# E-J408/admm-net

Measured on AMD Instinct MI355X. Metric: signals/sec (K-layer ADMM-Net forward), higher is better.
Workload: dtype f32; 1 GPU; cfg3: ADMMNet K=16 grid 16x16 (D=256, n=257) batch 65536/GPU + spectrum on 1024 atoms; batch_per_gpu=65536, global_batch=65536, K=16, D=256, n=257, natoms=1024, batch_mean_scope=global, chunk=8192, weights=torch.manual_seed(0) default init, glayer=matrix function, checked per matrix; eigensolver on the rejected matrices

## Files before the change

### admm_net_amd/csrc/spectral_fused.hip

```cpp
#include <stdio.h>
#include <stdlib.h>

#include <type_traits>

#include "common.h"
#include "rebuild_core.h"
#include "lane_reduce.h"

namespace admmnet {

constexpr int SF_THREADS = 768, SF_WAVES = 12;
constexpr int SF_PITCH = 40;
constexpr int SF_MAXM = 4;

typedef __bf16 bf16x8 __attribute__((ext_vector_type(8)));
typedef __bf16 bf16x2 __attribute__((ext_vector_type(2)));
typedef float f32x2v __attribute__((ext_vector_type(2)));
using f32x16 = __attribute__((ext_vector_type(16))) float;

__device__ __forceinline__ unsigned sf_pack_bf16(float a, float b) {
    const f32x2v p = {a, b};
    return __builtin_bit_cast(unsigned, __builtin_convertvector(p, bf16x2));
}
__device__ __forceinline__ float sf_bf16_lo(unsigned u) { return __uint_as_float(u << 16); }
__device__ __forceinline__ float sf_bf16_hi(unsigned u) { return __uint_as_float(u & 0xffff0000u); }

__device__ __forceinline__ float sf_reduce4(float a, float b, float c, float d) {
    float a2 = a, c2 = c, b2 = b, d2 = d;
    asm volatile("s_nop 1\n\tv_permlane32_swap_b32 %0, %1\n\tv_permlane32_swap_b32 %2, %3\n\ts_nop 1"
                 : "+v"(a2), "+v"(c2), "+v"(b2), "+v"(d2));
    float x = a2 + c2, y = b2 + d2;
    asm volatile("s_nop 1\n\tv_permlane16_swap_b32 %0, %1\n\ts_nop 1" : "+v"(x), "+v"(y));
    return pn_row16_sum(x + y);
}

template <int W>
__device__ __forceinline__ void sf_block_sum4(float &a, float &b, float &c, float &d, float *red ) {
    const float t = sf_reduce4(a, b, c, d);
    const int lane = threadIdx.x & 63, wave = threadIdx.x >> 6;
    __syncthreads();
    if ((lane & 15) == 0) red[(lane >> 4) * W + wave] = t;
    __syncthreads();
    float s[4];
#pragma unroll
    for (int q = 0; q < 4; ++q) {
        float v = 0.f;
#pragma unroll
        for (int w = 0; w < W; ++w) v += red[q * W + w];
        s[q] = v;
    }
    a = s[0]; b = s[1]; c = s[2]; d = s[3];
}

template <int W>
__device__ __forceinline__ void sf_block_sum8(float &a, float &b, float &c, float &d, float &e, float &f, float *red ) {
    const float t = sf_reduce4(a, b, c, d), u = sf_reduce4(e, f, 0.f, 0.f);
    const int lane = threadIdx.x & 63, wave = threadIdx.x >> 6;
    __syncthreads();
    if ((lane & 15) == 0) {
        red[(lane >> 4) * W + wave] = t;
        red[(4 + (lane >> 4)) * W + wave] = u;
    }
    __syncthreads();
    float s[6];
#pragma unroll
    for (int q = 0; q < 6; ++q) {
        float v = 0.f;
#pragma unroll
        for (int w = 0; w < W; ++w) v += red[q * W + w];
        s[q] = v;
    }
    a = s[0]; b = s[1]; c = s[2]; d = s[3]; e = s[4]; f = s[5];
}

struct SfCarve {
    int NP, NJ;
    float2 *X0, *X1, *Y0, *Y1, *ph, *Ob;
    float *hh, *hp, *red, *coef;
    double *sc;
    int *flags;
    float2 *part;
    unsigned short *ETre;
    unsigned short *ETim;
    __host__ __device__ static int np_of(int n) { return (n + 7) & ~7; }
    __host__ __device__ static int nj_of(int n) {
        const int D = n - 1, nt = (D + 31) >> 5;
        const int a = 32 * nt, b = (n + 7) & ~7;
        return a > b ? a : b;
    }
    __host__ __device__ static size_t bytes(int n, int W) {
        const size_t NP = np_of(n), NJ = nj_of(n);
        const size_t fixed = sizeof(float2) * 6 * NP + sizeof(float) * 2 * NP + sizeof(float) * 96 + sizeof(float) * 16 +
                             sizeof(double) * 16 + sizeof(int) * 4;
        const size_t part = sizeof(float2) * W * 2 * NP;
        const size_t slab = sizeof(unsigned short) * 2 * NJ * SF_PITCH;
        return fixed + (part > slab ? part : slab) + 64;
    }
    __device__ SfCarve(char *smem, int n) {
        NP = np_of(n);
        NJ = nj_of(n);
        sc = reinterpret_cast<double *>(smem);
        X0 = reinterpret_cast<float2 *>(sc + 16);
        X1 = X0 + NP; Y0 = X1 + NP; Y1 = Y0 + NP; ph = Y1 + NP; Ob = ph + NP;
        hh = reinterpret_cast<float *>(Ob + NP);
        hp = hh + NP;
        red = hp + NP;
        coef = red + 96;
        flags = reinterpret_cast<int *>(coef + 16);
        const int fixed = (int)(sizeof(double) * 16 + sizeof(float2) * 6 * NP + sizeof(float) * 2 * NP + sizeof(float) * 112 +
                                sizeof(int) * 4);
        char *u = smem + ((fixed + 15) & ~15);
        part = reinterpret_cast<float2 *>(u);
        ETre = reinterpret_cast<unsigned short *>(u);
        ETim = ETre + NJ * SF_PITCH;
    }
};

struct SfUpdate {
    const float *alpha;
    const float2 *phi_prev;
    const float *h_prev;
    const float *lw_prev;
    int mode;
};

__device__ __forceinline__ float2 sf_a_elem(int i, int j, int D, float2 z, float ir, float corner, float hi, float2 phj) {
    float2 a = make_float2(-ir * z.x, -ir * z.y);
    if (i < D) {
        if (i == j) a = make_float2(hi - ir * z.x, 0.f);
    } else {
        a = (j == D) ? make_float2(corner - ir * z.x, 0.f) : make_float2(phj.x - ir * z.x, -phj.y - ir * z.y);
    }
    return a;
}

template <int TPW, int W>
__global__ __launch_bounds__(64 * W, W == 12 ? 1 : 3) void sp_fused_kernel(int D, const float *__restrict__ lw, const float2 *__restrict__ phi,
                                                                 const float *__restrict__ h, float2 *Zg,
                                                                 float2 *G, float *__restrict__ rn,
                                                                 int *__restrict__ flag, int32_t *__restrict__ status, float tol,
                                                                 int iters, unsigned long long *__restrict__ ptime, SfUpdate up) {
    extern __shared__ __attribute__((aligned(16))) char smem[];
    long long t_prev = ptime ? clock64() : 0;
    auto mark = [&](int id) {
        if (ptime && threadIdx.x == 0) {
            const long long t_now = clock64();
            atomicAdd(&ptime[id], (unsigned long long)(t_now - t_prev));
            t_prev = t_now;
        }
    };
    const int n = D + 1;
    const SfCarve cv(smem, n);
    const int NP = cv.NP;
    const int64_t b = blockIdx.x;
    float2 *Z = Zg + b * (int64_t)n * n;
    const float2 *Gold = G + b * (int64_t)n * n;
    const int tid = threadIdx.x, lane = tid & 63;
    const int wave = __builtin_amdgcn_readfirstlane(tid >> 6);
    const float ir = lw[S_INV_RHO_G], corner = lw[S_CORNER_G];
    const int NT = (D + 31) >> 5, ntri = NT * (NT + 1) / 2;
    const int MM = (n + 63) >> 6;

    float pn = 0.f;
    if (tid < NP) {
        const float2 p = tid < D ? phi[b * D + tid] : make_float2(0.f, 0.f);
        cv.ph[tid] = p;
        cv.hh[tid] = tid < D ? h[b * D + tid] : 0.f;
        pn = p.x * p.x + p.y * p.y;
        if (up.mode) {
            cv.Ob[tid] = tid < D ? up.phi_prev[b * D + tid] : make_float2(0.f, 0.f);
            cv.hp[tid] = tid < D ? up.h_prev[b * D + tid] : 0.f;
        }
    }
    const float al = up.mode ? up.alpha[b] : 0.f;
    const float corner_zp = up.mode ? up.lw_prev[S_CORNER_Z] : 0.f;
    {
        float z1 = 0.f, z2 = 0.f, z3 = 0.f;
        sf_block_sum4<W>(pn, z1, z2, z3, cv.red);
    }
    const float ipn = pn > 0.f ? rsqrtf(pn) : 0.f;
    if (tid < NP) {
        const float2 p = cv.ph[tid];
        cv.X0[tid] = make_float2(tid == D ? 1.f : 0.f, 0.f);
        cv.X1[tid] = pn > 0.f ? make_float2(p.x * ipn, p.y * ipn) : make_float2(tid == 0 ? 1.f : 0.f, 0.f);
    }
    __syncthreads();

    mark(0);
    double trace = 0.0;
    float l0 = 0.f, l1 = 0.f, cf = 0.f, res0 = 0.f, res1 = 0.f;
    bool last = false;
    for (int it = 0; it < iters; ++it) {
        v2f x0[SF_MAXM], x1[SF_MAXM], c0[SF_MAXM], c1[SF_MAXM];
#pragma unroll
        for (int m = 0; m < SF_MAXM; ++m) {
            const int j = lane + 64 * m;
            const bool v = m < MM && j < n;
            x0[m] = v ? pk2(cv.X0[j]) : v2f{0.f, 0.f};
            x1[m] = v ? pk2(cv.X1[j]) : v2f{0.f, 0.f};
            c0[m] = v2f{0.f, 0.f};
            c1[m] = v2f{0.f, 0.f};
        }
        float trl = 0.f;
        auto run_pass = [&](auto updc) {
        constexpr bool UPD = decltype(updc)::value;
        float2 za[SF_MAXM], zb[SF_MAXM], zc[SF_MAXM], zd[SF_MAXM];
        float2 ga[SF_MAXM], gb[SF_MAXM], gc[SF_MAXM], gd[SF_MAXM];
        auto load_row = [&](int i, float2(&z)[SF_MAXM], float2(&g)[SF_MAXM]) {
#pragma unroll
            for (int m = 0; m < SF_MAXM; ++m) {
                const int j = lane + 64 * m;
                const bool v = i < n && j <= i;
                z[m] = (v && !(UPD && up.mode == 2)) ? Z[(int64_t)i * n + j] : make_float2(0.f, 0.f);
                if (UPD) g[m] = v ? Gold[(int64_t)i * n + j] : make_float2(0.f, 0.f);
            }
        };
        auto proc_row = [&](int i, float2(&zc)[SF_MAXM], const float2(&gq)[SF_MAXM]) {
            if (UPD) {
                const float hpi = cv.hp[i];
#pragma unroll
                for (int m = 0; m < SF_MAXM; ++m) {
                    if (64 * m <= i) {
                        const int j = lane + 64 * m;
                        if (j <= i) {
                            float2 c;
                            if (i < D) c = make_float2(i == j ? hpi : 0.f, 0.f);
                            else if (j == D) c = make_float2(corner_zp, 0.f);
                            else {
                                const float2 pp = cv.Ob[j];
                                c = make_float2(pp.x, -pp.y);
                            }
                            const float2 zn = make_float2(zc[m].x + al * (gq[m].x - c.x), zc[m].y + al * (gq[m].y - c.y));
                            zc[m] = zn;
                            Z[(int64_t)i * n + j] = zn;
                        }
                    }
                }
            }
            const v2f xi0 = pk2(cv.X0[i]), xi1 = pk2(cv.X1[i]);
            const float hi = cv.hh[i];
            v2f r0 = {0.f, 0.f}, r1 = {0.f, 0.f};
#pragma unroll
            for (int m = 0; m < SF_MAXM; ++m) {
                if (64 * m <= i) {
                    const int j = lane + 64 * m;
                    float2 a = sf_a_elem(i, j, D, zc[m], ir, corner, hi, (i == D && j < D) ? cv.ph[j] : make_float2(0.f, 0.f));
                    if (j > i) a = make_float2(0.f, 0.f);
                    if (j == i) trl += a.x;
                    const v2f av = pk2(a);
                    r0 = pk_cfma(r0, av, x0[m]);
                    r1 = pk_cfma(r1, av, x1[m]);
                    const v2f ac = (j < i) ? av : v2f{0.f, 0.f};
                    c0[m] = pk_cfma_conj(c0[m], ac, xi0);
                    c1[m] = pk_cfma_conj(c1[m], ac, xi1);
                }
            }
            if (i == 64 * SF_MAXM && lane == 0) {
                const int64_t idx = (int64_t)i * n + i;
                float2 z = (UPD && up.mode == 2) ? make_float2(0.f, 0.f) : Z[idx];
                if (UPD) {
                    const float2 g = Gold[idx];
                    z = make_float2(z.x + al * (g.x - corner_zp), z.y + al * g.y);
                    Z[idx] = z;
                }
                const float a = corner - ir * z.x;
                trl += a;
                const float2 xa = cv.X0[i], xb = cv.X1[i];
                r0.x += a * xa.x; r0.y += a * xa.y;
                r1.x += a * xb.x; r1.y += a * xb.y;
            }
            const float t = sf_reduce4(r0.x, r0.y, r1.x, r1.y);
            if ((lane & 15) == 0) {
                float *dst = reinterpret_cast<float *>((lane & 32) ? cv.Y1 : cv.Y0);
                dst[2 * i + ((lane >> 4) & 1)] = t;
            }
        };
        load_row(wave, za, ga);
        load_row(wave + W, zb, gb);
        for (int i = wave; i < n; i += 2 * W) {
            load_row(i + 2 * W, zc, gc);
            load_row(i + 3 * W, zd, gd);
            proc_row(i, za, ga);
            if (i + W < n) proc_row(i + W, zb, gb);
#pragma unroll
            for (int m = 0; m < SF_MAXM; ++m) {
                za[m] = zc[m];
                zb[m] = zd[m];
                ga[m] = gc[m];
                gb[m] = gd[m];
            }
        }
        };
        if (up.mode != 0 && it == 0) run_pass(std::true_type{});
        else run_pass(std::false_type{});
#pragma unroll
        for (int m = 0; m < SF_MAXM; ++m) {
            const int j = lane + 64 * m;
            if (m < MM && j < NP) {
                cv.part[(wave * 2 + 0) * NP + j] = make_float2(c0[m].x, c0[m].y);
                cv.part[(wave * 2 + 1) * NP + j] = make_float2(c1[m].x, c1[m].y);
            }
        }
        if (it == 0) {
            float z1 = 0.f, z2 = 0.f, z3 = 0.f;
            sf_block_sum4<W>(trl, z1, z2, z3, cv.red);
            trace = (double)trl;
        }
        __syncthreads();
        mark(1);
        float2 x0e = make_float2(0.f, 0.f), x1e = x0e, y0e = x0e, y1e = x0e;
        if (tid < n) {
            y0e = cv.Y0[tid];
            y1e = cv.Y1[tid];
#pragma unroll
            for (int w = 0; w < W; ++w) {
                if (tid >= 64 * SF_MAXM) break;
                const float2 p0 = cv.part[(w * 2 + 0) * NP + tid], p1 = cv.part[(w * 2 + 1) * NP + tid];
                y0e.x += p0.x; y0e.y += p0.y;
                y1e.x += p1.x; y1e.y += p1.y;
            }
            x0e = cv.X0[tid];
            x1e = cv.X1[tid];
        }
        float h00 = x0e.x * y0e.x + x0e.y * y0e.y, h11 = x1e.x * y1e.x + x1e.y * y1e.y;
        float h01r = x0e.x * y1e.x + x0e.y * y1e.y, h01i = x0e.x * y1e.y - x0e.y * y1e.x;
        sf_block_sum4<W>(h00, h11, h01r, h01i, cv.red);
        float ct = 1.f, st = 0.f, er = 1.f, ei = 0.f;
        {
            const float ab = sqrtf(h01r * h01r + h01i * h01i);
            const float dif = 0.5f * (h00 - h11), rad = sqrtf(dif * dif + ab * ab);
            l0 = 0.5f * (h00 + h11) - rad;
            l1 = 0.5f * (h00 + h11) + rad;
            const float vx = dif >= 0.f ? dif + rad : ab, vy = dif >= 0.f ? ab : rad - dif;
            const float nrm = sqrtf(vx * vx + vy * vy);
            if (nrm > 0.f) {
                ct = vx / nrm;
                st = vy / nrm;
            }
            if (ab > 0.f) {
                er = h01r / ab;
                ei = -h01i / ab;
            }
            cf = (float)((trace - (double)l0 - (double)l1) / (double)(n - 2));
            if (tid == 0) {
                cv.sc[0] = l0; cv.sc[1] = l1; cv.sc[2] = cf;
            }
        }
        const float2 ex1 = make_float2(er * x1e.x - ei * x1e.y, er * x1e.y + ei * x1e.x);
        const float2 ey1 = make_float2(er * y1e.x - ei * y1e.y, er * y1e.y + ei * y1e.x);
        const float2 nx0 = make_float2(-st * x0e.x + ct * ex1.x, -st * x0e.y + ct * ex1.y);
        const float2 nx1 = make_float2(ct * x0e.x + st * ex1.x, ct * x0e.y + st * ex1.y);
        const float2 ny0 = make_float2(-st * y0e.x + ct * ey1.x, -st * y0e.y + ct * ey1.y);
        const float2 ny1 = make_float2(ct * y0e.x + st * ey1.x, ct * y0e.y + st * ey1.y);
        const float2 d0 = make_float2(ny0.x - l0 * nx0.x, ny0.y - l0 * nx0.y);
        const float2 d1 = make_float2(ny1.x - l1 * nx1.x, ny1.y - l1 * nx1.y);
        float r0s = d0.x * d0.x + d0.y * d0.y, r1s = d1.x * d1.x + d1.y * d1.y;
        const float2 p0 = make_float2(ny0.x - cf * nx0.x, ny0.y - cf * nx0.y);
        const float2 p1 = make_float2(ny1.x - cf * nx1.x, ny1.y - cf * nx1.y);
        float n0 = p0.x * p0.x + p0.y * p0.y, n1 = p1.x * p1.x + p1.y * p1.y;
        float pr = p0.x * p1.x + p0.y * p1.y, pi = p0.x * p1.y - p0.y * p1.x;
        sf_block_sum8<W>(r0s, r1s, n0, n1, pr, pi, cv.red);
        res0 = sqrtf(r0s);
        res1 = sqrtf(r1s);
        last = it + 1 >= iters ||
               (it >= 1 && res0 <= 2e-6f * fabsf(l0 - cf) && res1 <= 2e-6f * fabsf(l1 - cf));
        if (!last) {
            const float in0 = n0 > 0.f ? rsqrtf(n0) : 0.f;
            const float2 q0 = make_float2(p0.x * in0, p0.y * in0);
            const float gr = pr * in0, gi = pi * in0;
            float2 q1 = make_float2(p1.x - (gr * q0.x - gi * q0.y), p1.y - (gr * q0.y + gi * q0.x));
            const float n1o = n1 - (gr * gr + gi * gi);
            const float in1 = n1o > 0.f ? rsqrtf(n1o) : 0.f;
            q1.x *= in1;
            q1.y *= in1;
            if (tid < NP) {
                cv.X0[tid] = tid < n ? q0 : make_float2(0.f, 0.f);
                cv.X1[tid] = tid < n ? q1 : make_float2(0.f, 0.f);
            }
        } else if (tid < NP) {
            cv.X0[tid] = tid < n ? nx0 : make_float2(0.f, 0.f);
            cv.X1[tid] = tid < n ? nx1 : make_float2(0.f, 0.f);
        }
        __syncthreads();
        mark(2);
        if (last) break;
    }
    const float mu0 = l0 - cf, mu1 = l1 - cf;

    int tI[TPW], tJ[TPW];
#pragma unroll
    for (int s = 0; s < TPW; ++s) tri_tile(wave * TPW + s, tI[s], tJ[s]);
    f32x16 accRe[TPW], accIm[TPW];
#pragma unroll
    for (int s = 0; s < TPW; ++s) {
#pragma unroll
        for (int q = 0; q < 16; ++q) {
            accRe[s][q] = 0.f;
            accIm[s][q] = 0.f;
        }
    }
    float2 ob = make_float2(0.f, 0.f);
    unsigned *ETre32 = reinterpret_cast<unsigned *>(cv.ETre), *ETim32 = reinterpret_cast<unsigned *>(cv.ETim);
    constexpr int P32 = SF_PITCH / 2;
    for (int idx = tid; idx < (cv.NJ - n) * P32; idx += (64 * W)) {
        ETre32[n * P32 + idx] = 0u;
        ETim32[n * P32 + idx] = 0u;
    }
    const int nslab = (n + 31) >> 5;
    for (int K = 0; K < nslab; ++K) {
        const int k0 = 32 * K;
        __syncthreads();
        int tl = tid;
        asm volatile("" : "+v"(tl));
        auto deflate = [&](float2 a, float2 vr0, float2 vc0, float2 vr1, float2 vc1, bool diag) {
            const float2 q0 = cmulc(vr0, vc0), q1 = cmulc(vr1, vc1);
            a.x -= mu0 * q0.x + mu1 * q1.x;
            a.y -= mu0 * q0.y + mu1 * q1.y;
            if (diag) {
                a.x -= cf;
                a.y = 0.f;
            }
            return a;
        };
        auto pair_of = [&](const float2 *v, int k, float2 &lo, float2 &hi) {
            const float4 t = *reinterpret_cast<const float4 *>(v + k);
            lo = make_float2(t.x, t.y);
            hi = make_float2(t.z, t.w);
        };
        {
            constexpr int RP = (64 * W) / 256, LQ = (16 + RP - 1) / RP;
            const int j = tl & 255;
            const float2 vj0 = cv.X0[j], vj1 = cv.X1[j], phj = cv.ph[j];
            constexpr int LB = 3;
#pragma unroll
            for (int qb = 0; qb < LQ; qb += LB) {
            float2 zl0[LB], zl1[LB];
#pragma unroll
            for (int uu = 0; uu < LB; ++uu) {
                const int kp = RP * (qb + uu) + (tl >> 8);
                const int k = k0 + 2 * kp;
                const bool v = kp < 16 && j <= k && j < n;
                zl0[uu] = (v && k < n) ? Z[(int64_t)k * n + j] : make_float2(0.f, 0.f);
                zl1[uu] = (v && k + 1 < n) ? Z[(int64_t)(k + 1) * n + j] : make_float2(0.f, 0.f);
            }
#pragma unroll
            for (int u = 0; u < LB; ++u) {
                const int kp = RP * (qb + u) + (tl >> 8);
                const int k = k0 + 2 * kp;
                if (kp < 16 && j <= k && j < n) {
                    float2 vk0, vk0b, vk1, vk1b;
                    pair_of(cv.X0, k, vk0, vk0b);
                    pair_of(cv.X1, k, vk1, vk1b);
                    const float2 hk = *reinterpret_cast<const float2 *>(cv.hh + k);
                    float2 e0 = make_float2(0.f, 0.f), e1 = e0;
                    if (k < n) e0 = deflate(sf_a_elem(k, j, D, zl0[u], ir, corner, hk.x, phj), vk0, vj0, vk1, vj1, k == j);
                    if (k + 1 < n) e1 = deflate(sf_a_elem(k + 1, j, D, zl1[u], ir, corner, hk.y, phj), vk0b, vj0, vk1b, vj1, k + 1 == j);
                    ETre32[j * P32 + kp] = sf_pack_bf16(e0.x, e1.x);
                    ETim32[j * P32 + kp] = sf_pack_bf16(e0.y, e1.y);
                }
            }
            }
        }
        if (tl < 16 && D >= 256) {
            const int kp = tl, k = k0 + 2 * kp, j = 256;
            if (j <= k && j < n) {
                float2 e0 = make_float2(0.f, 0.f);
                if (k < n)
                    e0 = deflate(sf_a_elem(k, j, D, Z[(int64_t)k * n + j], ir, corner, cv.hh[k], cv.ph[j]), cv.X0[k], cv.X0[j], cv.X1[k],
                                 cv.X1[j], k == j);
                ETre32[j * P32 + kp] = sf_pack_bf16(e0.x, 0.f);
                ETim32[j * P32 + kp] = sf_pack_bf16(e0.y, 0.f);
            }
        }
        {
            constexpr int RPS = (64 * W) / 16, UB = 2;
            const int kp = tl & 15, k = k0 + 2 * kp;
            const int kc = k < NP - 1 ? k : 0;
            float2 vk0, vk0b, vk1, vk1b, phk, phkb;
            pair_of(cv.X0, kc, vk0, vk0b);
            pair_of(cv.X1, kc, vk1, vk1b);
            pair_of(cv.ph, kc, phk, phkb);
            for (int jb = k0 + 1; jb < n; jb += UB * RPS) {
                float2 zu0[UB], zu1[UB];
#pragma unroll
                for (int u = 0; u < UB; ++u) {
                    const int j = jb + RPS * u + (tl >> 4);
                    const bool v = j < n && j >= k + 1;
                    zu0[u] = v ? Z[(int64_t)j * n + k] : make_float2(0.f, 0.f);
                    zu1[u] = (v && k + 1 < n) ? Z[(int64_t)j * n + k + 1] : make_float2(0.f, 0.f);
                }
#pragma unroll
                for (int u = 0; u < UB; ++u) {
                    const int j = jb + RPS * u + (tl >> 4);
                    if (j < n && j >= k + 1) {
                        const float hj = cv.hh[j];
                        const float2 vj0 = cv.X0[j], vj1 = cv.X1[j];
                        float2 e0 = deflate(sf_a_elem(j, k, D, zu0[u], ir, corner, hj, phk), vj0, vk0, vj1, vk1, false);
                        float2 e1 = make_float2(0.f, 0.f);
                        if (k + 1 < n)
                            e1 = deflate(sf_a_elem(j, k + 1, D, zu1[u], ir, corner, hj, phkb), vj0, vk0b, vj1, vk1b, j == k + 1);
                        ETre32[j * P32 + kp] = sf_pack_bf16(e0.x, e1.x);
                        ETim32[j * P32 + kp] = sf_pack_bf16(-e0.y, -e1.y);
                    }
                }
            }
        }
        __syncthreads();
        mark(3);
        {
            int r32 = lane & 31, kh = lane >> 5;
            asm volatile("" : "+v"(r32), "+v"(kh));
#pragma unroll
            for (int ks = 0; ks < 2; ++ks) {
                const int off = 8 * ks + 4 * kh;
                uint4 are = make_uint4(0, 0, 0, 0), aim = are;
#pragma unroll
                for (int s = 0; s < TPW; ++s) {
                    if (wave * TPW + s < ntri) {
                        const int ia = 32 * tI[s] + r32, jb_ = 32 * tJ[s] + r32;
                        if (s == 0 || tI[s] != tI[s - 1]) {
                            are = *reinterpret_cast<const uint4 *>(ETre32 + ia * P32 + off);
                            aim = *reinterpret_cast<const uint4 *>(ETim32 + ia * P32 + off);
                        }
                        const uint4 bre = *reinterpret_cast<const uint4 *>(ETre32 + jb_ * P32 + off);
                        const uint4 bim = *reinterpret_cast<const uint4 *>(ETim32 + jb_ * P32 + off);
                        const uint4 nbre = make_uint4(bre.x ^ 0x80008000u, bre.y ^ 0x80008000u, bre.z ^ 0x80008000u,
                                                      bre.w ^ 0x80008000u);
                        const bf16x8 Are = __builtin_bit_cast(bf16x8, are), Aim = __builtin_bit_cast(bf16x8, aim);
                        const bf16x8 Bre = __builtin_bit_cast(bf16x8, bre), Bim = __builtin_bit_cast(bf16x8, bim);
                        const bf16x8 nBre = __builtin_bit_cast(bf16x8, nbre);
                        accRe[s] = __builtin_amdgcn_mfma_f32_32x32x16_bf16(Are, Bre, accRe[s], 0, 0, 0);
                        accIm[s] = __builtin_amdgcn_mfma_f32_32x32x16_bf16(Are, Bim, accIm[s], 0, 0, 0);
                        accRe[s] = __builtin_amdgcn_mfma_f32_32x32x16_bf16(Aim, Bim, accRe[s], 0, 0, 0);
                        accIm[s] = __builtin_amdgcn_mfma_f32_32x32x16_bf16(Aim, nBre, accIm[s], 0, 0, 0);
                    }
                }
            }
        }
        mark(4);
        __syncthreads();
        if (tid < n) {
            const unsigned *dre = ETre32 + D * P32, *dim = ETim32 + D * P32;
            const unsigned *jre = ETre32 + tid * P32, *jim = ETim32 + tid * P32;
#pragma unroll 2
            for (int kp = 0; kp < 16; ++kp) {
                const unsigned ur = dre[kp], ui = dim[kp], vr = jre[kp], vi = jim[kp];
                const float ar0 = sf_bf16_lo(ur), ai0 = sf_bf16_lo(ui), br0 = sf_bf16_lo(vr), bi0 = sf_bf16_lo(vi);
                const float ar1 = sf_bf16_hi(ur), ai1 = sf_bf16_hi(ui), br1 = sf_bf16_hi(vr), bi1 = sf_bf16_hi(vi);
                {
                    asm volatile("v_fma_f32 %0, %1, %2, %0" : "+v"(ob.x) : "v"(ar0), "v"(br0));
                    asm volatile("v_fma_f32 %0, %1, %2, %0" : "+v"(ob.x) : "v"(ai0), "v"(bi0));
                    asm volatile("v_fma_f32 %0, %1, %2, %0" : "+v"(ob.x) : "v"(ar1), "v"(br1));
                    asm volatile("v_fma_f32 %0, %1, %2, %0" : "+v"(ob.x) : "v"(ai1), "v"(bi1));
                    asm volatile("v_fma_f32 %0, %1, %2, %0" : "+v"(ob.y) : "v"(ar0), "v"(bi0));
                    asm volatile("v_fma_f32 %0, -%1, %2, %0" : "+v"(ob.y) : "v"(ai0), "v"(br0));
                    asm volatile("v_fma_f32 %0, %1, %2, %0" : "+v"(ob.y) : "v"(ar1), "v"(bi1));
                    asm volatile("v_fma_f32 %0, -%1, %2, %0" : "+v"(ob.y) : "v"(ai1), "v"(br1));
                }
            }
        }
        mark(5);
    }
    __syncthreads();
    if (tid < NP) cv.Ob[tid] = tid < n ? ob : make_float2(0.f, 0.f);

    float fro = 0.f;
    {
        const int r32 = lane & 31, kh = lane >> 5;
#pragma unroll
        for (int s = 0; s < TPW; ++s) {
            if (wave * TPW + s < ntri) {
                const float wgt = tI[s] == tJ[s] ? 1.f : 2.f;
                const int gj = 32 * tJ[s] + r32;
#pragma unroll
                for (int q = 0; q < 16; ++q) {
                    const int gi = 32 * tI[s] + (q & 3) + 8 * (q >> 2) + 4 * kh;
                    if (gi < D && gj < D) fro += wgt * (accRe[s][q] * accRe[s][q] + accIm[s][q] * accIm[s][q]);
                }
            }
        }
        if (tid < n) fro += (tid < D ? 2.f : 1.f) * (ob.x * ob.x + ob.y * ob.y);
        float z1 = 0.f, z2 = 0.f, z3 = 0.f;
        sf_block_sum4<W>(fro, z1, z2, z3, cv.red);
    }
    const LayerLayout L{D};
    const float *vn = lw + L.off_vn();
    if (wave == 0) {
        const double thr = lw[S_THR];
        const double dl0 = cv.sc[0], dl1 = cv.sc[1], c = cv.sc[2];
        const double delta = sqrt(sqrt((double)fro)) * (1.0 + 0x1p-8);
        const double ts[9] = {-1.0, 0.0, 1.0, -0.75, -0.5, -0.25, 0.25, 0.5, 0.75};
        double arg = c;
        if (lane < 9) arg = c + ts[lane] * delta;
        else if (lane == 9) arg = dl0;
        else if (lane == 10) arg = dl1;
        const double fv = eig_map_f64(arg, thr, vn);
        auto bcast = [&](int src) {
            const long long bits = __builtin_bit_cast(long long, fv);
            const int lo = __builtin_amdgcn_readlane((int)(bits & 0xffffffffll), src);
            const int hi = __builtin_amdgcn_readlane((int)(bits >> 32), src);
            return __builtin_bit_cast(double, ((long long)hi << 32) | (unsigned long long)(unsigned)lo);
        };
        const double fm = bcast(0), fc = bcast(1), fp = bcast(2), f0k = bcast(9), f1k = bcast(10);
        const double a0 = fc, a1 = (fp - fm) / (2.0 * delta), a2 = (fp - 2.0 * fc + fm) / (2.0 * delta * delta);
        const double scale = fmax(fmax(fabs(fc), fmax(fabs(f0k), fabs(f1k))), 1e-6);
        double miss = 0.0;
        if (lane >= 3 && lane < 9) {
            const double t = ts[lane] * delta;
            miss = fabs(fv - (a0 + a1 * t + a2 * t * t));
        }
#pragma unroll
        for (int o = 8; o > 0; o >>= 1) miss = fmax(miss, __shfl_xor(miss, o, 64));
        if (lane == 0) {
            int why = 0;
            const double g0 = fabs(dl0 - c), g1 = fabs(dl1 - c);
            if (!(isfinite(dl0) && isfinite(dl1) && isfinite(c) && isfinite(delta) && delta > 0.0 && isfinite(miss))) why = 8;
            else if (!((double)res0 <= 1e-5 * fmax(g0, 1e-30) && (double)res1 <= 1e-5 * fmax(g1, 1e-30))) why = 1;
            else if (!(delta < 0.05 * fmin(g0, g1))) why = 2;
            else if (!(miss <= (double)tol * scale)) why = 4;
            else if (!(fabs(a2) * delta * delta <= 1e-4 * scale)) why = 16;
            cv.coef[0] = (float)(a0 - a1 * c);
            cv.coef[1] = (float)a1;
            cv.coef[2] = (float)a2;
            cv.coef[3] = (float)(f0k - a0 - a1 * (dl0 - c));
            cv.coef[4] = (float)(f1k - a0 - a1 * (dl1 - c));
            cv.flags[0] = why;
            flag[b] = why;
            if (status) {
                atomicAdd(status + (why ? 1 : 2), 1);
                if (why == 4) atomicAdd(status + 3, 1);
            }
        }
    }
    __syncthreads();
    mark(6);
    if (cv.flags[0]) return;

    const float k0c = cv.coef[0], a1f = cv.coef[1], a2f = cv.coef[2], g0f = cv.coef[3], g1f = cv.coef[4];
    const float corner_z = lw[S_CORNER_Z];
    float2 *Gb = G + b * (int64_t)n * n;
    float acc = 0.f;
    {
        const int r32 = lane & 31, kh = lane >> 5;
#pragma unroll
        for (int s = 0; s < TPW; ++s) {
            if (wave * TPW + s < ntri) {
                const int gj = 32 * tJ[s] + r32;
                const float2 vj0 = cv.X0[gj < n ? gj : 0], vj1 = cv.X1[gj < n ? gj : 0];
                constexpr int AB = 16;
#pragma unroll
                for (int qb = 0; qb < 16; qb += AB) {
                    float2 zq[AB];
#pragma unroll
                    for (int u = 0; u < AB; ++u) {
                        const int q = qb + u, gi = 32 * tI[s] + (q & 3) + 8 * (q >> 2) + 4 * kh;
                        zq[u] = (gi < D && gj <= gi) ? Z[(int64_t)gi * n + gj] : make_float2(0.f, 0.f);
                    }
#pragma unroll
                    for (int u = 0; u < AB; ++u) {
                        const int q = qb + u, gi = 32 * tI[s] + (q & 3) + 8 * (q >> 2) + 4 * kh;
                        if (gi < D && gj <= gi) {
                            const float hi = cv.hh[gi];
                            const float2 a = sf_a_elem(gi, gj, D, zq[u], ir, corner, hi, make_float2(0.f, 0.f));
                            const float2 p0 = cmulc(cv.X0[gi], vj0), p1 = cmulc(cv.X1[gi], vj1);
                            float2 g = make_float2(a1f * a.x + a2f * accRe[s][q] + g0f * p0.x + g1f * p1.x,
                                                   a1f * a.y + a2f * accIm[s][q] + g0f * p0.y + g1f * p1.y);
                            float cz = 0.f;
                            if (gi == gj) {
                                g.x += k0c;
                                g.y = 0.f;
                                cz = hi;
                            }
                            Gb[(int64_t)gi * n + gj] = g;
                            const float dr = g.x - cz;
                            acc += (gi == gj ? 1.f : 2.f) * (dr * dr + g.y * g.y);
                        }
                    }
                }
            }
        }
    }
    if (tid < n) {
        const int j = tid;
        const float2 a = sf_a_elem(D, j, D, Z[(int64_t)D * n + j], ir, corner, 0.f, cv.ph[j]);
        const float2 o = cv.Ob[j];
        const float2 p0 = cmulc(cv.X0[D], cv.X0[j]), p1 = cmulc(cv.X1[D], cv.X1[j]);
        float2 g = make_float2(a1f * a.x + a2f * o.x + g0f * p0.x + g1f * p1.x, a1f * a.y + a2f * o.y + g0f * p0.y + g1f * p1.y);
        float2 cz = make_float2(cv.ph[j].x, -cv.ph[j].y);
        if (j == D) {
            g.x += k0c;
            g.y = 0.f;
            cz = make_float2(corner_z, 0.f);
        }
        Gb[(int64_t)D * n + j] = g;
        const float dr = g.x - cz.x, di = g.y - cz.y;
        acc += (j == D ? 1.f : 2.f) * (dr * dr + di * di);
    }
    {
        float z1 = 0.f, z2 = 0.f, z3 = 0.f;
        sf_block_sum4<W>(acc, z1, z2, z3, cv.red);
    }
    if (tid == 0) rn[b] = sqrtf(acc);
    mark(7);
}

template <int TPW, int W>
static int sf_launch(int D, int64_t nb, const float *lw, const float2 *phi, const float *h, float2 *Z, float2 *G, float *rn,
                     int *flag, int32_t *status, float tol, int iters, bool timing, const SfUpdate &up, hipStream_t st) {
    const size_t lds = SfCarve::bytes(D + 1, W);
    ADMM_HIP(hipFuncSetAttribute(reinterpret_cast<const void *>(sp_fused_kernel<TPW, W>), hipFuncAttributeMaxDynamicSharedMemorySize,
                                 (int)lds));
    PhaseTimer tm;
    if (int rc = tm.begin(timing, st, 16)) return rc;
    hipLaunchKernelGGL((sp_fused_kernel<TPW, W>), dim3((unsigned)nb), dim3(64 * W), lds, st, D, lw, phi, h, Z, G, rn, flag, status,
                       tol, iters, tm.dev, up);
    ADMM_HIP(hipGetLastError());
    if (tm.dev) {
        unsigned long long hb[16];
        if (int rc = tm.end(st, hb)) return rc;
        fprintf(stderr, "[sf timing D=%d nb=%lld] cycles per workgroup: setup %.0f | matvec %.0f ritz %.0f (all passes) | stage %.0f "
                "mfma %.0f border %.0f (all slabs) | model %.0f | assemble %.0f\n", D, (long long)nb, hb[0] / (double)nb,
                hb[1] / (double)nb, hb[2] / (double)nb, (hb[3]) / (double)nb, hb[4] / (double)nb, hb[5] / (double)nb,
                hb[6] / (double)nb, hb[7] / (double)nb);
    }
    return ADMMNET_OK;
}

static_assert(SF_WAVES == 12, "spectral_waves (route.h) names the shapes 4 and 12");

int launch_spectral_fused(const Switches &sw, int D, int64_t nb, const float *lw, const float2 *phi, const float *h, float2 *Z,
                          float2 *G, float *rn, int *flag, int32_t *status, const float *alpha, const float2 *phi_prev,
                          const float *h_prev, const float *lw_prev, int update_mode, int waves, hipStream_t st) {
    const SfUpdate up{alpha, phi_prev, h_prev, lw_prev, update_mode};
    if (D < 2 || D > 256) {
        set_error("spectral: D=%d outside 2..256", D);
        return ADMMNET_E_ARG;
    }
    if (!(waves == SF_WAVES || (waves == 4 && D <= 128))) {
        set_error("spectral: %d waves per matrix at D=%d (need 12, or 4 with D <= 128)", waves, D);
        return ADMMNET_E_ARG;
    }
    const float tol = sw.spectral_tol;
    const int iters = sw.spectral_iters;
    const bool timing = sw.sf_timing;
    const int NT = (D + 31) >> 5, ntri = NT * (NT + 1) / 2;
    if (waves == 4) {
        switch ((ntri + 3) / 4) {
            case 1: return sf_launch<1, 4>(D, nb, lw, phi, h, Z, G, rn, flag, status, tol, iters, timing, up, st);
            case 2: return sf_launch<2, 4>(D, nb, lw, phi, h, Z, G, rn, flag, status, tol, iters, timing, up, st);
            default: return sf_launch<3, 4>(D, nb, lw, phi, h, Z, G, rn, flag, status, tol, iters, timing, up, st);
        }
    }
    switch ((ntri + SF_WAVES - 1) / SF_WAVES) {
        case 1: return sf_launch<1, SF_WAVES>(D, nb, lw, phi, h, Z, G, rn, flag, status, tol, iters, timing, up, st);
        case 2: return sf_launch<2, SF_WAVES>(D, nb, lw, phi, h, Z, G, rn, flag, status, tol, iters, timing, up, st);
        default: return sf_launch<3, SF_WAVES>(D, nb, lw, phi, h, Z, G, rn, flag, status, tol, iters, timing, up, st);
    }
}

}
```

Measured before the change: 92800 signals/s.

## Restructure spectral row pipeline with clamped unpredicated loads and fewer registers

The row-streaming pass now uses clamped row and column indices, so loads are unconditional instead of predicated. A 4-deep software pipeline replaces the 2-deep one with a separate tail loop, and the per-wave array width shrinks to 3 when W=4. Loads are split into update and no-Z-load template variants, and 32-bit address arithmetic plus asm barriers are used to control register pressure and the placement of memory operations. The goal is to cut predication overhead and VGPR use in the main power-iteration and G-rebuild loops. The risks are redundant clamped loads and the need for the NM=3 width to stay correct for W=4 configurations. An ISA summary profiling script is also added.

```diff
diff --git a/admm_net_amd/csrc/spectral_fused.hip b/admm_net_amd/csrc/spectral_fused.hip
--- a/admm_net_amd/csrc/spectral_fused.hip
+++ b/admm_net_amd/csrc/spectral_fused.hip
@@ -134,6 +134,18 @@
     return a;
 }
 
+__device__ __forceinline__ int sf_tri_row(int i, int n) { return i < n ? i : n - 1; }
+__device__ __forceinline__ unsigned sf_tri_col(unsigned j, unsigned i) { return j < i ? j : i; }
+__device__ __forceinline__ float2 sf_keep(bool v, float2 z) { return v ? z : make_float2(0.f, 0.f); }
+__device__ __forceinline__ float2 sf_tri_load(const float2 *Z, int n, int i, int j) {
+    const unsigned ic = sf_tri_row(i, n), jc = sf_tri_col(j, ic);
+    return *reinterpret_cast<const float2 *>(reinterpret_cast<const char *>(Z) + (ic * (unsigned)n + jc) * 8u);
+}
+
+__device__ __forceinline__ float2 *sf_elem(float2 *M, int n, int i, int j) {
+    return reinterpret_cast<float2 *>(reinterpret_cast<char *>(M) + ((unsigned)i * (unsigned)n + (unsigned)j) * 8u);
+}
+
 template <int TPW, int W>
 __global__ __launch_bounds__(64 * W, W == 12 ? 1 : 3) void sp_fused_kernel(int D, const float *__restrict__ lw, const float2 *__restrict__ phi,
                                                                  const float *__restrict__ h, float2 *Zg,
@@ -190,7 +202,11 @@
     double trace = 0.0;
     float l0 = 0.f, l1 = 0.f, cf = 0.f, res0 = 0.f, res1 = 0.f;
     bool last = false;
+    const int tid_k = tid;
     for (int it = 0; it < iters; ++it) {
+        int tid_o = tid_k;
+        asm volatile("" : "+v"(tid_o));
+        const int tid = tid_o, lane = tid & 63;
         v2f x0[SF_MAXM], x1[SF_MAXM], c0[SF_MAXM], c1[SF_MAXM];
 #pragma unroll
         for (int m = 0; m < SF_MAXM; ++m) {
@@ -202,49 +218,52 @@
             c1[m] = v2f{0.f, 0.f};
         }
         float trl = 0.f;
-        auto run_pass = [&](auto updc) {
+        constexpr int NM = W == 4 ? 3 : SF_MAXM;
+        auto run_pass = [&](auto updc, auto zldc) {
         constexpr bool UPD = decltype(updc)::value;
-        float2 za[SF_MAXM], zb[SF_MAXM], zc[SF_MAXM], zd[SF_MAXM];
-        float2 ga[SF_MAXM], gb[SF_MAXM], gc[SF_MAXM], gd[SF_MAXM];
-        auto load_row = [&](int i, float2(&z)[SF_MAXM], float2(&g)[SF_MAXM]) {
-#pragma unroll
-            for (int m = 0; m < SF_MAXM; ++m) {
-                const int j = lane + 64 * m;
-                const bool v = i < n && j <= i;
-                z[m] = (v && !(UPD && up.mode == 2)) ? Z[(int64_t)i * n + j] : make_float2(0.f, 0.f);
-                if (UPD) g[m] = v ? Gold[(int64_t)i * n + j] : make_float2(0.f, 0.f);
+        constexpr bool ZLD = decltype(zldc)::value;
+        float2 za[NM], zb[NM], zc[NM], zd[NM];
+        float2 ga[NM], gb[NM], gc[NM], gd[NM];
+#pragma unroll
+        for (int m = 0; m < NM; ++m) zc[m] = zd[m] = gc[m] = gd[m] = make_float2(0.f, 0.f);
+        auto load_row = [&](int i, float2(&z)[NM], float2(&g)[NM]) {
+            const int ic = sf_tri_row(i, n);
+            const float2 *zr = Z + (int64_t)ic * n, *gr = Gold + (int64_t)ic * n;
+#pragma unroll
+            for (int m = 0; m < NM; ++m) {
+                const unsigned jc = sf_tri_col(lane + 64 * m, ic);
+                z[m] = ZLD ? zr[jc] : make_float2(0.f, 0.f);
+                if (UPD) g[m] = gr[jc];
             }
         };
-        auto proc_row = [&](int i, float2(&zc)[SF_MAXM], const float2(&gq)[SF_MAXM]) {
+        auto proc_row = [&](int i, float2(&zc)[NM], const float2(&gq)[NM], auto cornc) {
             if (UPD) {
                 const float hpi = cv.hp[i];
-#pragma unroll
-                for (int m = 0; m < SF_MAXM; ++m) {
-                    if (64 * m <= i) {
-                        const int j = lane + 64 * m;
-                        if (j <= i) {
-                            float2 c;
-                            if (i < D) c = make_float2(i == j ? hpi : 0.f, 0.f);
-                            else if (j == D) c = make_float2(corner_zp, 0.f);
-                            else {
-                                const float2 pp = cv.Ob[j];
-                                c = make_float2(pp.x, -pp.y);
-                            }
-                            const float2 zn = make_float2(zc[m].x + al * (gq[m].x - c.x), zc[m].y + al * (gq[m].y - c.y));
-                            zc[m] = zn;
-                            Z[(int64_t)i * n + j] = zn;
-                        }
+                float2 *zw = Z + (int64_t)i * n;
+#pragma unroll
+                for (int m = 0; m < NM; ++m) {
+                    const int jc = (int)sf_tri_col(lane + 64 * m, i);
+                    float2 c;
+                    if (i < D) c = make_float2(i == jc ? hpi : 0.f, 0.f);
+                    else if (jc == D) c = make_float2(corner_zp, 0.f);
+                    else {
+                        const float2 pp = cv.Ob[jc];
+                        c = make_float2(pp.x, -pp.y);
                     }
+                    const float2 zn = make_float2(zc[m].x + al * (gq[m].x - c.x), zc[m].y + al * (gq[m].y - c.y));
+                    zc[m] = zn;
+                    zw[(unsigned)jc] = zn;
                 }
             }
             const v2f xi0 = pk2(cv.X0[i]), xi1 = pk2(cv.X1[i]);
             const float hi = cv.hh[i];
             v2f r0 = {0.f, 0.f}, r1 = {0.f, 0.f};
 #pragma unroll
-            for (int m = 0; m < SF_MAXM; ++m) {
+            for (int m = 0; m < NM; ++m) {
                 if (64 * m <= i) {
                     const int j = lane + 64 * m;
-                    float2 a = sf_a_elem(i, j, D, zc[m], ir, corner, hi, (i == D && j < D) ? cv.ph[j] : make_float2(0.f, 0.f));
+                    const float2 zv = sf_keep(j <= i, zc[m]);
+                    float2 a = sf_a_elem(i, j, D, zv, ir, corner, hi, (i == D && j < D) ? cv.ph[j] : make_float2(0.f, 0.f));
                     if (j > i) a = make_float2(0.f, 0.f);
                     if (j == i) trl += a.x;
                     const v2f av = pk2(a);
@@ -255,9 +274,9 @@
                     c1[m] = pk_cfma_conj(c1[m], ac, xi1);
                 }
             }
-            if (i == 64 * SF_MAXM && lane == 0) {
+            if (W == SF_WAVES && decltype(cornc)::value && i == 64 * SF_MAXM && lane == 0) {
                 const int64_t idx = (int64_t)i * n + i;
-                float2 z = (UPD && up.mode == 2) ? make_float2(0.f, 0.f) : Z[idx];
+                float2 z = ZLD ? Z[idx] : make_float2(0.f, 0.f);
                 if (UPD) {
                     const float2 g = Gold[idx];
                     z = make_float2(z.x + al * (g.x - corner_zp), z.y + al * g.y);
@@ -275,24 +294,34 @@
                 dst[2 * i + ((lane >> 4) & 1)] = t;
             }
         };
-        load_row(wave, za, ga);
-        load_row(wave + W, zb, gb);
-        for (int i = wave; i < n; i += 2 * W) {
+        const int nmain = n < 64 * SF_MAXM ? n : 64 * SF_MAXM;
+        int i = wave;
+        load_row(i, za, ga);
+        load_row(i + W, zb, gb);
+        for (; i + 3 * W < nmain; i += 4 * W) {
             load_row(i + 2 * W, zc, gc);
             load_row(i + 3 * W, zd, gd);
-            proc_row(i, za, ga);
-            if (i + W < n) proc_row(i + W, zb, gb);
-#pragma unroll
-            for (int m = 0; m < SF_MAXM; ++m) {
-                za[m] = zc[m];
-                zb[m] = zd[m];
-                ga[m] = gc[m];
-                gb[m] = gd[m];
+            proc_row(i, za, ga, std::false_type{});
+            proc_row(i + W, zb, gb, std::false_type{});
+            load_row(i + 4 * W, za, ga);
+            load_row(i + 5 * W, zb, gb);
+            proc_row(i + 2 * W, zc, gc, std::false_type{});
+            proc_row(i + 3 * W, zd, gd, std::false_type{});
+        }
+        if (i + 2 * W < n) load_row(i + 2 * W, zc, gc);
+        for (; i < n; i += W) {
+            proc_row(i, za, ga, std::true_type{});
+            if (i + 3 * W < n) load_row(i + 3 * W, zd, gd);
+#pragma unroll
+            for (int m = 0; m < NM; ++m) {
+                za[m] = zb[m]; zb[m] = zc[m]; zc[m] = zd[m];
+                ga[m] = gb[m]; gb[m] = gc[m]; gc[m] = gd[m];
             }
         }
         };
-        if (up.mode != 0 && it == 0) run_pass(std::true_type{});
-        else run_pass(std::false_type{});
+        if (up.mode == 0 || it != 0) run_pass(std::false_type{}, std::true_type{});
+        else if (up.mode == 2) run_pass(std::true_type{}, std::false_type{});
+        else run_pass(std::true_type{}, std::true_type{});
 #pragma unroll
         for (int m = 0; m < SF_MAXM; ++m) {
             const int j = lane + 64 * m;
@@ -654,8 +683,10 @@
 #pragma unroll
                     for (int u = 0; u < AB; ++u) {
                         const int q = qb + u, gi = 32 * tI[s] + (q & 3) + 8 * (q >> 2) + 4 * kh;
-                        zq[u] = (gi < D && gj <= gi) ? Z[(int64_t)gi * n + gj] : make_float2(0.f, 0.f);
+                        zq[u] = sf_tri_load(Z, n, gi, gj);
                     }
+#pragma unroll
+                    for (int u = 0; u < AB; ++u) asm volatile("" : "+v"(zq[u].x), "+v"(zq[u].y));
 #pragma unroll
                     for (int u = 0; u < AB; ++u) {
                         const int q = qb + u, gi = 32 * tI[s] + (q & 3) + 8 * (q >> 2) + 4 * kh;
@@ -671,7 +702,7 @@
                                 g.y = 0.f;
                                 cz = hi;
                             }
-                            Gb[(int64_t)gi * n + gj] = g;
+                            *sf_elem(Gb, n, gi, gj) = g;
                             const float dr = g.x - cz;
                             acc += (gi == gj ? 1.f : 2.f) * (dr * dr + g.y * g.y);
                         }
diff --git a/profiles/r13/isa_summary.py b/profiles/r13/isa_summary.py
--- /dev/null
+++ b/profiles/r13/isa_summary.py
@@ -0,0 +1,115 @@
+import re
+import sys
+
+EVENT = re.compile(r"^\s+(global_load\w*|global_store\w*|global_atomic\w*|scratch_load\w*|scratch_store\w*|s_barrier|"
+                   r"s_cbranch_\w+|s_branch|v_mfma\w*|s_waitcnt)\b(.*)$")
+LABEL = re.compile(r"^(\.LBB\d+_\d+):")
+META = ("vgpr_count", "agpr_count", "sgpr_count", "vgpr_spill_count", "private_segment_fixed_size", "group_segment_fixed_size",
+        "max_flat_workgroup_size")
+
+
+def kernels(text):
+    out = {}
+    lines = text.splitlines()
+    starts = [(i, m) for i, l in enumerate(lines)
+              for m in [re.match(r"^(_ZN7admmnet15sp_fused_kernelILi(\d+)ELi(\d+)EE\w+):", l)] if m]
+    for i, m in starts:
+        end = next(j for j in range(i, len(lines)) if lines[j].startswith(".Lfunc_end"))
+        out[(int(m.group(2)), int(m.group(3)))] = [lines[i:end], {}, m.group(1)]
+    blocks, cur = [], None
+    for l in lines:
+        if re.match(r"^  - \.\w+:", l):
+            cur = {}
+            blocks.append(cur)
+        m = re.match(r"^\s+(?:- )?\.(\w+):\s+(\S+)\s*$", l)
+        if m and cur is not None:
+            cur[m.group(1)] = m.group(2)
+    for blk in blocks:
+        for k in out.values():
+            if k[2] == blk.get("name"):
+                k[1].update({key: int(blk[key]) for key in META if key in blk})
+    return out
+
+
+def occupancy(meta):
+    regs = (meta["vgpr_count"] + meta.get("agpr_count", 0) + 7) // 8 * 8
+    waves = min(8, 512 // regs)
+    per_simd = meta["max_flat_workgroup_size"] // 64 // 4 or 1
+    return waves, waves // per_simd
+
+
+def events(body):
+    ev = []
+    for l in body:
+        m = LABEL.match(l)
+        if m:
+            ev.append(("label", m.group(1)))
+            continue
+        m = EVENT.match(l)
+        if not m:
+            continue
+        op, rest = m.group(1), m.group(2)
+        if op == "s_waitcnt":
+            v = re.search(r"vmcnt\((\d+)\)", rest)
+            if v:
+                ev.append(("wait", "vmcnt(%s)" % v.group(1)))
+        elif op.startswith("s_cbranch") or op == "s_branch":
+            ev.append(("branch", "%s %s" % (op, rest.strip())))
+        else:
+            ev.append(("mem" if not op.startswith(("s_barrier", "v_mfma")) else "op", op))
+    return ev
+
+
+def collapse(ev):
+    out = []
+    for kind, what in ev:
+        if out and kind in ("mem", "op") and out[-1][0] == kind and out[-1][1] == what:
+            out[-1][2] += 1
+        else:
+            out.append([kind, what, 1])
+    return out
+
+
+def loops(ev):
+    pos = {what: i for i, (kind, what) in enumerate(ev) if kind == "label"}
+    spans = []
+    for i, (kind, what) in enumerate(ev):
+        if kind == "branch":
+            tgt = what.split()[-1]
+            if tgt in pos and pos[tgt] < i:
+                spans.append((pos[tgt], i))
+    return [s for s in spans if not any(o != s and s[0] <= o[0] and o[1] <= s[1] for o in spans)]
+
+
+def show(ev):
+    for kind, what, cnt in collapse(ev):
+        if kind == "label":
+            print("%s:" % what)
+        elif kind == "branch":
+            print("      %s" % what)
+        else:
+            print("    %s%s" % ("%d x " % cnt if cnt > 1 else "", what))
+
+
+def main():
+    text = open(sys.argv[1]).read()
+    ks = kernels(text)
+    print("| kernel | VGPRs | spilled | scratch bytes | static LDS | waves / SIMD | workgroups / CU |")
+    print("|---|---|---|---|---|---|---|")
+    for key in sorted(ks, key=lambda k: (k[1], k[0])):
+        meta = ks[key][1]
+        w, g = occupancy(meta)
+        print("| `<%d, %d>` | %d | %d | %d | %d | %d | %d |" % (key[0], key[1], meta["vgpr_count"], meta["vgpr_spill_count"],
+                                                               meta["private_segment_fixed_size"], meta["group_segment_fixed_size"], w, g))
+    if len(sys.argv) >= 4:
+        ev = events(ks[(int(sys.argv[2]), int(sys.argv[3]))][0])
+        if "--loops" in sys.argv:
+            for a, b in loops(ev):
+                print("-- loop %s" % ev[a][1])
+                show(ev[a:b + 1])
+        else:
+            show(ev)
+
+
+if __name__ == "__main__":
+    main()
```

Result: faster. 95080 signals/s (median of 6 runs) (+2.5%).
